# NTU-CompHydroMet-Lab/P2I-GAN-benchmark

Measured on AMD Instinct MI355X. Metric: train frames/sec (128x128x16), higher is better.
Workload: dtype f32

## Files before the change

include/p2i_hip.h:

```cpp
#ifndef P2I_HIP_H
#define P2I_HIP_H
#include <stdint.h>

#ifdef __cplusplus
extern "C" {
#endif

#define P2I_OK 0
#define P2I_EINVAL (-1)
#define P2I_ELDS (-2)

#define P2I_ACT_NONE 0
#define P2I_ACT_RELU 1
#define P2I_ACT_LEAKY 2
#define P2I_ACT_TANH 3

int p2i_abi_version(void);
const char* p2i_last_error(void);

typedef struct {
  int B, Cin, Cout;
  int Ti, Hi, Wi;
  int To, Ho, Wo;
  int kt, kh, kw;
  int st, sh, sw;
  int pt, ph, pw;
} p2i_conv_desc;

int p2i_conv_fwd(const p2i_conv_desc* d, const float* x, const float* wp, const float* bias,
                 const float* residual, float* y, int act, void* stream);
int p2i_conv_dgrad(const p2i_conv_desc* d, const float* dy, const float* y_act, int act,
                   const float* wp_d, const float* dx_add, const float* mask_y, int mask_act,
                   float* dx, void* stream);
int p2i_conv_wgrad(const p2i_conv_desc* d, const float* x, const float* dy, const float* y_act,
                   int act, float* dwp, float* dbias, void* stream);
int p2i_conv_wgrad_ws(const p2i_conv_desc* d, const float* x, const float* dy, const float* y_act, int act, float* dwp,
                      float* dbias, float* ws, int64_t ws_floats, void* stream);
int p2i_conv_fwd_x6(const p2i_conv_desc* d, const float* x, const float* wp, uint16_t* wsplit, const float* bias,
                    const float* residual, float* y, int act, void* stream);
int p2i_conv_dgrad_x6(const p2i_conv_desc* d, const float* dy, const float* wp_d, uint16_t* wsplit, const float* dx_add,
                      const float* mask_y, int mask_act, float* dx, void* stream);
int p2i_x6_split(const float* wp, uint16_t* wb, int ntaps, int K, int Mpad, void* stream);
int p2i_x6_split_batched(const float* const* wp, uint16_t* const* wb, const int* ntaps, const int* K, const int* Mpad, int n,
                         void* stream);
int p2i_x6c_would_take(const p2i_conv_desc* d, int dgrad, int act);
int p2i_conv_fwd_x6s(const p2i_conv_desc* d, const float* x, const float* wp, const uint16_t* wb_layer, int ntaps_w,
                     const float* bias, const float* residual, float* y, int act, void* stream);
int p2i_conv_dgrad_x6s(const p2i_conv_desc* d, const float* dy, const float* wp_d, const uint16_t* wb_layer, int ntaps_w,
                       const float* dx_add, const float* mask_y, int mask_act, float* dx, void* stream);
int p2i_conv_last_plan(int* out6);
int p2i_fast_div_magic(int d, uint32_t* magic);
int p2i_wgrad_last_plan(int* out4);

int p2i_doconv_fold_fwd(const float* W, const float* D, const float* D_diag, int O, int I, int groups,
                        int ksz, int identity_rep, float* wp_f, float* wp_d, void* stream);
int p2i_doconv_fold_bwd(const float* dwp_f, const float* W, const float* D, const float* D_diag,
                        int O, int I, int groups, int ksz, float* dW, float* dD, void* stream);

int p2i_doconv_fold_fwd_batched(const float* const* W, const float* const* D, const float* const* D_diag, int n, int O, int I,
                                float* const* wp_f, float* const* wp_d, void* stream);
int p2i_doconv_fold_bwd_batched(const float* const* dwp_f, const float* const* W, const float* const* D,
                                const float* const* D_diag, int n, int O, int I, float* const* dW, float* const* dD,
                                void* stream);

int p2i_weight_pack(const float* w, int O, int I, int ntaps, const float* inv_div_ptr,
                    float* wp_f, float* wp_d, void* stream);
int p2i_weight_unpack_grad(const float* dwp_f, int O, int I, int ntaps, const float* w_orig,
                           const float* sigma_ptr, const float* u, const float* v, float* scratch,
                           float* dw, void* stream);

int p2i_weight_pack_batched(const float* const* w, const int* O, const int* I, const int* ntaps, const float* const* inv_div,
                            float* const* wp_f, float* const* wp_d, int n, void* stream);
int p2i_weight_unpack_grad_batched(const float* const* dwp_f, const int* O, const int* I, const int* ntaps,
                                   const float* const* w_orig, const float* const* sigma, const float* const* u,
                                   const float* const* v, float* dots, float* const* dw, int n, void* stream);

int p2i_weight_unpack_grad_batched_acc(const float* const* dwp_f, const int* O, const int* I, const int* ntaps,
                                       const float* const* w_orig, const float* const* sigma, const float* const* u,
                                       const float* const* v, float* dots, float* const* dw, int n, int accumulate, void* stream);

int p2i_spectral_norm(const float* w, int O, int K, float* u, float* v, int training, float* sigma,
                      float* scratch, void* stream);

int p2i_spectral_norm_batched(const float* const* w, const int* O, const int* K, float* const* u, float* const* v,
                              int training, float* const* sigma, float* const* scratch, float* const* u_snap,
                              float* const* v_snap, int n, void* stream);

int p2i_attn_fwd(const float* x, const float* w0, const float* b0, const float* w1, const float* b1,
                 float* out, int B, int T, int HW, void* stream);
int p2i_attn_bwd(const float* x, const float* w0, const float* b0, const float* w1, const float* b1,
                 const float* dout, float* dw0, float* db0, float* dw1, float* db1,
                 int B, int T, int HW, void* stream);

int p2i_idw_fwd(const float* vals_src, const float* mask, const float* grid_x, const float* grid_y,
                const float* grid_z, float* out, int32_t* pt_pos, int32_t* pt_count, int32_t* frame_count,
                int32_t* row_start, float* pt_xyzn, int32_t* sel_idx, float* sel_w, int B, int T, int H, int W, float tau,
                void* stream);
int p2i_idw_fwd_ws(const float* vals_src, const float* mask, const float* grid_x, const float* grid_y,
                   const float* grid_z, float* out, int32_t* pt_pos, int32_t* pt_count, int32_t* frame_count,
                   int32_t* row_start, float* pt_xyzn, int32_t* sel_idx, float* sel_w, int32_t* amb, int B, int T, int H, int W,
                   float tau, void* stream);
int p2i_idw_bwd(const float* dout, const int32_t* pt_pos, const int32_t* pt_count, const int32_t* sel_idx,
                const float* sel_w, float* dvals_src, int B, int T, int H, int W, void* stream);

int p2i_pooldup_fwd(const float* x, float* y, int B, int C, int H, int W, void* stream);
int p2i_pooldup_bwd(const float* x, const float* dy, float* dx, int B, int C, int H, int W, void* stream);

int p2i_upmod_fwd(const float* x, const float* pos, float* u, int B, int C, int S, int S2w , void* stream);
int p2i_upmod_fwd_ba(const float* v, const float* pos, const float* bias, int act, float* u, int B, int C, int S, int S2w, void* stream);
int p2i_upmod_bwd(const float* x, const float* pos, const float* du, float* dx, float* dpos,
                  int B, int C, int S, int S2w, void* stream);

int p2i_dtail_fwd(const float* out2d, const float* out3d, const float* alpha2d, float* fused,
                  int B, int H2, int W2, int T3, int H3, int W3, void* stream);
int p2i_dtail_bwd(const float* out2d, const float* alpha2d, const float* dfused, float* dout2d,
                  float* dout3d, float* dalpha2d, int B, int H2, int W2, int T3, int H3, int W3, void* stream);

int p2i_recloss(const float* pred, const float* target, float k1_alpha, float* out3, float* dpred,
                float* scratch, int B, int T, int HW, void* stream);
int p2i_gan_loss(const float* logits_a, const float* logits_b, int n, int loss_type, int mode,
                 float weight, float real_label, float fake_label, float* loss, float* dlogits_a,
                 float* dlogits_b, void* stream);

int p2i_adam(float* p, const float* g, float* m, float* v, int64_t n, float lr, float beta1,
             float beta2, float eps, int step, void* stream);

int p2i_assemble_batch(const uint8_t* frames_u8, const uint8_t* mask_u8, int64_t mask_numel, float* frames,
                       float* masked, float* masks, int B, int T, int H, int W, void* stream);

int p2i_window_gather(const float* a, const float* b , float* wa, float* wb, int L, int64_t HW, int w0, int nw, int win,
                      int step, void* stream);
int p2i_window_mean(const float* pred_windows, float* out, int L, int64_t HW, int nwin, int win, int step, float scale, void* stream);

// ... 78 lines not shown
```

p2i-gan-benchmark_amd/csrc/conv.hip:

```cpp
#include "conv_dma.h"

namespace p2i {


template <int MB, int NPIX, int WAVES_M, int CK>
__global__ __launch_bounds__(256) void patch_gemm_kernel(const PatchGeom g) {
  extern __shared__ __attribute__((aligned(16))) float smem[];
  constexpr int WAVES_N = 4 / WAVES_M;
  constexpr int TM = MB / (32 * WAVES_M);
  constexpr int TN = NPIX / (32 * WAVES_N);
  static_assert(TM >= 1 && TN >= 1, "tile too small");
  float* lw = smem;
  float* lp = smem + g.ntaps * CK * MB;

  const int tid = threadIdx.x, lane = tid & 63, wave = tid >> 6;
  const int wm = wave / WAVES_N, wn = wave % WAVES_N;
  const int l31 = lane & 31, lhi = lane >> 5;

  int tile = blockIdx.x;
  const int tw = tile % g.ntw; tile /= g.ntw;
  const int th = tile % g.nth; tile /= g.nth;
  const int tt = tile % g.ntt;
  const int tb = tile / g.ntt;
  const int j0b = tb << g.ljb, j0t = tt << g.ljt, j0h = th << g.ljh, j0w = tw << g.ljw;
// ... 76 lines not shown
        for (int i = 0; i < TM; ++i)
#pragma unroll
          for (int f = 0; f < TN; ++f)
            acc[i][f] = __builtin_amdgcn_mfma_f32_32x32x2f32(a[i], bv[f], acc[i][f], 0, 0, 0);
      }
    }
  }

  const int dHW = g.dH * g.dW;
#pragma unroll
  for (int f = 0; f < TN; ++f) {
    const int pix = (wn * TN + f) * 32 + l31;
    const int gw = j0w + (pix & JWm);
    const int gh = j0h + ((pix >> g.ljw) & JHm);
    const int gt = j0t + ((pix >> (g.ljw + g.ljh)) & JTm);
    const int gb = j0b + (pix >> (g.ljw + g.ljh + g.ljt));
    const bool pv = gb < g.B && gt < g.nT && gh < g.nH && gw < g.nW;
    const int sp = (gt * g.oT + g.pT) * dHW + (gh * g.oH + g.pH) * g.dW + gw * g.oW + g.pW;
#pragma unroll
    for (int i = 0; i < TM; ++i) {
#pragma unroll
      for (int r = 0; r < 16; ++r) {
        const int o = o0 + (wm * TM + i) * 32 + (r & 3) + 8 * (r >> 2) + 4 * lhi;
        if (pv && o < g.Cm) {
          float v = acc[i][f][r];
          if (g.bias) v += g.bias[o];
          v = act_apply(v, g.act_epi);
          const size_t di = ((size_t)(gb * g.Cm + o)) * g.dT * dHW + sp;
          if (g.res) v += g.res[di];
          if (g.mask_y) v = act_grad(v, g.mask_y[di], g.mask_act);
          g.dst[di] = v;
        }
      }
    }
  }
}


typedef void (*patch_fn)(const PatchGeom);
template <int MB, int NPIX, int WM, int CK>
static int launch_patch(const PatchGeom& g, dim3 grid, size_t lds, hipStream_t s) {
  auto k = patch_gemm_kernel<MB, NPIX, WM, CK>;
  static bool attr_set = false;
  if (!attr_set) {
    (void)hipFuncSetAttribute((const void*)k, hipFuncAttributeMaxDynamicSharedMemorySize, 160 * 1024);
    attr_set = true;
  }
  P2I_LAUNCH(k, grid, dim3(256), lds, s, g);
  return launch_status();
}

static int dispatch_patch_dma(const TileCfg& c, int KG, const PatchGeom& g, dim3 grid, size_t lds, hipStream_t s) {
  int rc = dispatch_patch_dma_g0(c, KG, g, grid, lds, s);
  if (rc == -1) rc = dispatch_patch_dma_g1(c, KG, g, grid, lds, s);
  if (rc == -1) rc = dispatch_patch_dma_g2(c, KG, g, grid, lds, s);
  if (rc == -1) rc = dispatch_patch_dma_g3(c, KG, g, grid, lds, s);
  if (rc != -1) return rc;
  set_error("no DMA kernel instance for tile cfg %d %d %d %d kg %d", c.MB, c.NPIX, c.WM, c.CK, KG);
  return P2I_EINVAL;
}

static int dispatch_patch(const TileCfg& c, const PatchGeom& g, dim3 grid, size_t lds, hipStream_t s) {
#define P2I_CASE(mb_, npix_, wm_, ck_) \
  if (c.MB == mb_ && c.NPIX == npix_ && c.WM == wm_ && c.CK == ck_) return launch_patch<mb_, npix_, wm_, ck_>(g, grid, lds, s);
  P2I_CASE(128, 256, 2, 8)
  P2I_CASE(64, 256, 1, 8)
  P2I_CASE(64, 128, 2, 8)
  P2I_CASE(32, 128, 1, 8)
  P2I_CASE(128, 256, 2, 4)
  P2I_CASE(64, 256, 1, 4)
  P2I_CASE(64, 128, 2, 4)
  P2I_CASE(32, 128, 1, 4)
  P2I_CASE(128, 256, 2, 2)
  P2I_CASE(64, 256, 1, 2)
  P2I_CASE(64, 128, 2, 2)
  P2I_CASE(32, 128, 1, 2)
#undef P2I_CASE
  set_error("no kernel instance for tile cfg %d %d %d %d", c.MB, c.NPIX, c.WM, c.CK);
  return P2I_EINVAL;
}


static thread_local int g_last_plan[6] = {0, 0, 0, 0, 0, 0};

static int run_patch_gemm(PatchGeom g, const ClassSpec& cs, hipStream_t s);

static int run_patch_gemm_classes(PatchGeom g, const ClassSpec* css, int ncls, hipStream_t s) {
  if (g.src_y != nullptr || ncls > MAX_CLASSES) return 1;
  if (const X6Ctx& xc = x6_ctx(); xc.wb != nullptr) {
    bool all = true;
    for (int q = 0; q < ncls && all; ++q) all = run_patch_gemm_x6c(g, css[q], xc.wb, xc.ntaps_w, nullptr, s, true) == 0;
    if (all) {
      for (int q = 0; q < ncls; ++q)
        if (const int rc = run_patch_gemm_x6c(g, css[q], xc.wb, xc.ntaps_w, g_last_plan, s)) return rc == 1 ? P2I_EINVAL : rc;
      return P2I_OK;
    }
  }
  const ClassSpec& c0s = css[0];
  g.mT = c0s.mT; g.mH = c0s.mH; g.mW = c0s.mW;
  g.oT = c0s.oT; g.oH = c0s.oH; g.oW = c0s.oW;
  int lo[MAX_CLASSES][3], rng[3] = {0, 0, 0}, mx[3] = {0, 0, 0}, max_taps = 0;
  long long total_pix = 0;
  for (int q = 0; q < ncls; ++q) {
    const ClassSpec& cs = css[q];
    int hi[3] = {0, 0, 0};
    lo[q][0] = lo[q][1] = lo[q][2] = 0;
    for (int i = 0; i < cs.ntaps; ++i) {
      const int d[3] = {cs.dt[i], cs.dh[i], cs.dw[i]};
      for (int k = 0; k < 3; ++k) {
        if (i == 0 || d[k] < lo[q][k]) lo[q][k] = d[k];
        if (i == 0 || d[k] > hi[k]) hi[k] = d[k];
      }
    }
    for (int k = 0; k < 3; ++k) if (hi[k] - lo[q][k] > rng[k]) rng[k] = hi[k] - lo[q][k];
    if (cs.nT > mx[0]) mx[0] = cs.nT;
    if (cs.nH > mx[1]) mx[1] = cs.nH;
    if (cs.nW > mx[2]) mx[2] = cs.nW;
    if (cs.ntaps > max_taps) max_taps = cs.ntaps;
    total_pix += (long long)g.B * (cs.nT > 0 ? cs.nT : 0) * (cs.nH > 0 ? cs.nH : 0) * (cs.nW > 0 ? cs.nW : 0);
  }
  if (mx[0] <= 0 || mx[1] <= 0 || mx[2] <= 0) return P2I_OK;
  if (max_taps == 0) max_taps = 1;
  g.ntaps = max_taps;
  static const int cand[5][3] = {{128, 256, 2}, {64, 256, 1}, {128, 128, 2}, {64, 128, 2}, {32, 128, 1}};
  int best = -1, best_ck = 0;
  long long best_score = -1;
  PatchGeom bg = g;
  size_t best_lds = 0;
  dim3 best_grid;
  for (int ci = 0; ci < 5; ++ci) {
    const int MBc = cand[ci][0], NP = cand[ci][1];
    if (MBc > 32 && g.Cm <= MBc / 2) continue;
    int jb, jt, jh, jw;
    pick_tile_dims(NP, g.B, mx[0], mx[1], mx[2], jb, jt, jh, jw);
    PatchGeom t = g;
    t.ljb = ilog2(jb); t.ljt = ilog2(jt); t.ljh = ilog2(jh); t.ljw = ilog2(jw);
    t.eT = (jt - 1) * g.mT + rng[0] + 1;
    t.eH = patch_extent_div((jh - 1) * g.mH + rng[1] + 1);
    t.eW = (jw - 1) * g.mW + rng[2] + 1;
    bool same_lo_w = true;
    for (int q = 1; q < ncls; ++q) same_lo_w = same_lo_w && lo[q][2] == lo[0][2];
    t.v4 = (conv_v4_on() && same_lo_w && (g.sW & 3) == 0 && ((jw * g.mW) & 3) == 0) ? 1 : 0;
    t.v4sh = 0;
    if (t.v4) {
      t.v4sh = ((lo[0][2] % 4) + 4) % 4;
      t.eW = (t.eW + t.v4sh + 3) & ~3;
      t.eW4 = t.eW >> 2;
    }
    if (!t.v4) t.eW = patch_extent_div(t.eW);
    t.eWp = t.eW;
    t.eth = t.eT * t.eH;
    t.rpc = jb * t.eth;
    t.CSl = t.rpc * t.eW;
    t.CS = t.CSl;
    t.G4 = t.CSl >> 2;
    const int force_ck16 = P2I_ENV_ONCE("P2I_CONV_CK16", 0);
    for (int CKc = ((max_taps <= 4 || ((force_ck16 || g.Ck >= 256) && max_taps == 9 && MBc <= 64)) ? 16 : 8); CKc >= 2; CKc >>= 1) {
      if (g.Ck >= CKc ? (g.Ck % CKc != 0) : (CKc != 2 && g.Ck * 2 <= CKc)) continue;
      if (CKc == 2 && !(MBc == 64 && NP == 128) && !(MBc == 32)) continue;
      if ((CKc == 4 || CKc == 16) && MBc == 128 && NP == 128) continue;
      const int PT = CKc * t.CSl;
      if (PT >= 65536 || t.CSl >= 65536) continue;
      const int PTp = t.v4 ? (((PT >> 2) + 63) & ~63) * 4 : (PT + 63) & ~63;
      const int nwrows = max_taps * CKc;
      const size_t WSZ = (size_t)((nwrows * (MBc / 4) + 63) & ~63) * 4;
      const size_t lds = sizeof(float) * (((nwrows + 63) & ~63) + (size_t)PTp + 2 * (WSZ + PTp));
      if (lds > 160 * 1024) continue;
      const long long nb = (long long)ceil_div(g.Cm, MBc) * ((total_pix + NP - 1) / NP);
      long long score = (nb >= 256 ? 1000000000ll : nb * 1000000ll) + (long long)MBc * NP * 10 + CKc + (lds <= 80 * 1024 ? 5 : 0);
      if (score > best_score) {
        best_score = score; best = ci; best_ck = CKc; best_lds = lds;
        bg = t; bg.PT = PT;
        bg.ntt = ceil_div(mx[0], jt); bg.nth = ceil_div(mx[1], jh); bg.ntw = ceil_div(mx[2], jw);
        best_grid = dim3((unsigned)(ceil_div(g.B, jb) * bg.ntt * bg.nth * bg.ntw), (unsigned)ceil_div(g.Cm, MBc), (unsigned)ncls);
      }
      break;
    }
  }
  const unsigned long long sbytes = 4ull * g.B * g.Ck * g.sT * g.sH * g.sW;
  if (best < 0 || sbytes >= 0xF0000000ull) return 1;
  TileCfg c{cand[best][0], cand[best][1], cand[best][2], best_ck};
  P2I_REQUIRE(magic_u16_ok(bg.CSl) && magic_u16_ok(bg.eW) && magic_u16_ok(bg.rpc) && magic_u16_ok(bg.eth) && magic_u16_ok(bg.eH) &&
              (!bg.v4 || (magic_u16_ok(bg.G4) && (bg.eW4 == 1 || magic_u16_ok(bg.eW4)))),
              "conv planner: offset-table divisor outside [2, 65535] (%d %d %d %d %d)", bg.CSl, bg.eW, bg.rpc, bg.eth, bg.eH);
  bg.mg_csl = magic_u16(bg.CSl); bg.mg_ew = magic_u16(bg.eW);
  bg.mg_rpc = magic_u16(bg.rpc); bg.mg_eth = magic_u16(bg.eth); bg.mg_eh = magic_u16(bg.eH);
  if (bg.v4) { bg.mg_g4 = magic_u16(bg.G4); bg.mg_ew4 = magic_u16(bg.eW4); }
  bg.src_bytes = (unsigned)sbytes;
  bg.wp_bytes = g.wp_bytes;
  bg.nclass = ncls;
  for (int q = 0; q < ncls; ++q) {
    const ClassSpec& cs = css[q];
    ClassGeom& cgm = bg.cls[q];
    cgm.nT = cs.nT; cgm.nH = cs.nH; cgm.nW = cs.nW;
    cgm.pT = cs.pT; cgm.pH = cs.pH; cgm.pW = cs.pW;
    cgm.bT = lo[q][0]; cgm.bH = lo[q][1]; cgm.bW = lo[q][2];
    cgm.ntaps = cs.ntaps;
    for (int i = 0; i < cs.ntaps; ++i) {
      cgm.tap_w[i] = cs.tw[i];
      cgm.tap_off[i] = ((cs.dt[i] - lo[q][0]) * bg.eH + (cs.dh[i] - lo[q][1])) * bg.eW + (cs.dw[i] - lo[q][2]);
    }
  }
  bg.nT = css[0].nT; bg.nH = css[0].nH; bg.nW = css[0].nW;
  bg.pT = css[0].pT; bg.pH = css[0].pH; bg.pW = css[0].pW;
  bg.bT = lo[0][0]; bg.bH = lo[0][1]; bg.bW = lo[0][2];
  for (int i = 0; i < css[0].ntaps; ++i) { bg.tap_w[i] = bg.cls[0].tap_w[i]; bg.tap_off[i] = bg.cls[0].tap_off[i]; }
  if (bg.v4) {
    bg.bW -= bg.v4sh;
    for (int i = 0; i < css[0].ntaps; ++i) bg.tap_off[i] += bg.v4sh;
    for (int q = 0; q < ncls; ++q) {
      bg.cls[q].bW -= bg.v4sh;
      for (int i = 0; i < css[q].ntaps; ++i) bg.cls[q].tap_off[i] += bg.v4sh;
    }
  }
  if (ncls == 1) bg.ntaps = css[0].ntaps;
  const long long nb = (long long)best_grid.x * best_grid.y * best_grid.z;
  const int acc_regs = (c.MB / 32) * (c.NPIX / 32) / 4 * 16;
  const size_t red_bytes = (size_t)4 * acc_regs * 64 * 4;
  const int kg27 = P2I_ENV_ONCE("P2I_CONV_KG27", 1);
  const bool kg_27 = kg27 && max_taps == 27 && c.CK == 4 && ncls == 1;
  const int KG = ((nb <= 320 || (c.CK == 16 && max_taps == 9) || kg_27) && (c.CK >= 8 || kg_27) && c.MB <= 64 && red_bytes <= best_lds) ? 2 : 1;
  g_last_plan[0] = c.MB; g_last_plan[1] = c.NPIX; g_last_plan[2] = c.WM; g_last_plan[3] = c.CK;
  g_last_plan[4] = ncls > 1 ? 0 : ((max_taps == 9 && (c.CK <= 8 || KG == 2)) ? 9 : (max_taps == 1 ? 1 : ((max_taps == 27 && (c.CK == 4 || (c.CK < 4 && KG == 1))) ? 27 : 0)));
  g_last_plan[5] = KG;
  return dispatch_patch_dma(c, KG, bg, best_grid, best_lds, s);
}

static int run_patch_gemm(PatchGeom g, const ClassSpec& cs, hipStream_t s) {
  if (cs.nT <= 0 || cs.nH <= 0 || cs.nW <= 0) return P2I_OK;
  {
    const int rc = run_patch_gemm_classes(g, &cs, 1, s);
    if (rc != 1) return rc;
  }
  g.nT = cs.nT; g.nH = cs.nH; g.nW = cs.nW;
  g.mT = cs.mT; g.mH = cs.mH; g.mW = cs.mW;
  g.oT = cs.oT; g.oH = cs.oH; g.oW = cs.oW; g.pT = cs.pT; g.pH = cs.pH; g.pW = cs.pW;
  g.ntaps = cs.ntaps;
  g.nclass = 1;
  int lo[3] = {0, 0, 0}, hi[3] = {0, 0, 0};
  for (int i = 0; i < cs.ntaps; ++i) {
    const int d[3] = {cs.dt[i], cs.dh[i], cs.dw[i]};
    for (int k = 0; k < 3; ++k) {
      if (i == 0 || d[k] < lo[k]) lo[k] = d[k];
      if (i == 0 || d[k] > hi[k]) hi[k] = d[k];
    }
  }
  g.bT = lo[0]; g.bH = lo[1]; g.bW = lo[2];

  TileCfg c;
  c.CK = (g.Ck == 1) ? 2 : (cs.ntaps > 9 ? 4 : 8);
  if (g.Ck < c.CK && g.Ck > 1) c.CK = (g.Ck >= 4) ? 4 : 2;
  c.MB = g.Cm > 64 ? 128 : (g.Cm > 32 ? 64 : 32);
  c.NPIX = 256;
  const long long total_pix = (long long)g.B * cs.nT * cs.nH * cs.nW;
  auto nblocks = [&](const TileCfg& t) { return (long long)ceil_div(g.Cm, t.MB) * ((total_pix + t.NPIX - 1) / t.NPIX); };
  const long long want = 512;
  while (nblocks(c) < want) {
    if (c.MB == 128) { c.MB = 64; continue; }
    if (c.NPIX == 256) { c.NPIX = 128; continue; }
    if (c.MB == 64 && g.Cm > 32) { c.MB = 32; continue; }
    break;
  }
  if (c.MB == 128) { c.NPIX = 256; c.WM = 2; }
  else if (c.MB == 64) { c.WM = (c.NPIX == 256) ? 1 : 2; }
  else { c.NPIX = 128; c.WM = 1; }

  for (int attempt = 0; attempt < 4; ++attempt) {
    int jb, jt, jh, jw;
    pick_tile_dims(c.NPIX, g.B, cs.nT, cs.nH, cs.nW, jb, jt, jh, jw);
    g.ljb = ilog2(jb); g.ljt = ilog2(jt); g.ljh = ilog2(jh); g.ljw = ilog2(jw);
    g.eT = (jt - 1) * cs.mT + (hi[0] - lo[0]) + 1;
    g.eH = patch_extent_div((jh - 1) * cs.mH + (hi[1] - lo[1]) + 1);
    g.eW = (jw - 1) * cs.mW + (hi[2] - lo[2]) + 1;
    g.eWp = g.eW | 1;
    g.eth = g.eT * g.eH;
    g.rpc = jb * g.eth;
    g.CS = g.rpc * g.eWp;
    P2I_REQUIRE(magic_u16_ok(g.eH) && magic_u16_ok(g.eth) && g.rpc >= 2, "conv planner: staging divisor below 2 (%d %d %d)", g.rpc, g.eth, g.eH);
    g.mg_rpc = magic_u16(g.rpc); g.mg_eth = magic_u16(g.eth); g.mg_eh = magic_u16(g.eH);
    const size_t lds = sizeof(float) * ((size_t)cs.ntaps * c.CK * c.MB + (size_t)c.CK * g.CS);
    if (lds > 160 * 1024 || c.CK * g.rpc >= 65536) {
      if (c.CK > 2) { c.CK /= 2; continue; }
      if (c.NPIX == 256) { c.NPIX = 128; c.WM = (c.MB == 64) ? 2 : (c.MB == 128 ? 2 : 1); if (c.MB == 128) c.MB = 64; continue; }
      set_error("conv tile does not fit LDS (%zu bytes)", lds);
      return P2I_ELDS;
    }
    for (int i = 0; i < cs.ntaps; ++i) {
      g.tap_w[i] = cs.tw[i];
      g.tap_off[i] = ((cs.dt[i] - lo[0]) * g.eH + (cs.dh[i] - lo[1])) * g.eWp + (cs.dw[i] - lo[2]);
    }
    g.ntt = ceil_div(cs.nT, jt); g.nth = ceil_div(cs.nH, jh); g.ntw = ceil_div(cs.nW, jw);
    const int ntb = ceil_div(g.B, jb);
    dim3 grid((unsigned)(ntb * g.ntt * g.nth * g.ntw), (unsigned)ceil_div(g.Cm, c.MB));
    g_last_plan[0] = c.MB; g_last_plan[1] = c.NPIX; g_last_plan[2] = c.WM; g_last_plan[3] = c.CK; g_last_plan[4] = -1; g_last_plan[5] = 0;
    return dispatch_patch(c, g, grid, lds, s);
  }
  set_error("conv tile selection failed");
  return P2I_ELDS;
}

}

using namespace p2i;

#ifdef P2I_STAMP
namespace p2i { __device__ unsigned long long* p2i_stamp_buf = nullptr; }
extern "C" int p2i_debug_set_stamp(unsigned long long* buf) {
  return (int)hipMemcpyToSymbol(HIP_SYMBOL(p2i::p2i_stamp_buf), &buf, sizeof(buf));
}
#endif

extern "C" int p2i_conv_last_plan(int* out6) {
  if (!out6) return P2I_EINVAL;
  for (int i = 0; i < 6; ++i) out6[i] = g_last_plan[i];
  return P2I_OK;
}

extern "C" int p2i_fast_div_magic(int d, uint32_t* magic) {
  P2I_REQUIRE(magic != nullptr, "null pointer");
  P2I_REQUIRE(magic_u16_ok(d), "fast_div: no 32-bit multiplier for divisor %d (2 <= d < 65536)", d);
  *magic = magic_u16(d);
  return P2I_OK;
}

extern "C" int p2i_conv_fwd(const p2i_conv_desc* d, const float* x, const float* wp, const float* bias,
                            const float* residual, float* y, int act, void* stream) {
  if (int e = check_desc(d)) return e;
  P2I_REQUIRE(x && wp && y, "null pointer");
  if (d->Cin == 1 && residual == nullptr && x6_ctx().wb == nullptr) {
    const int rc = c1_fwd(d, x, wp, bias, y, act, (hipStream_t)stream);
    if (rc != 1) { g_last_plan[0] = 32; g_last_plan[1] = 64; g_last_plan[2] = 1; g_last_plan[3] = 2; g_last_plan[4] = 27; g_last_plan[5] = 1; return rc; }
  }
  if (d->Cout == 1 && residual == nullptr) {
    const int rc = o1_fwd(d, x, wp, bias, y, act, (hipStream_t)stream);
    if (rc != 1) { g_last_plan[0] = 1; g_last_plan[1] = 64; g_last_plan[2] = 8; g_last_plan[3] = 1; g_last_plan[4] = 9; g_last_plan[5] = 3; return rc; }
  }
  PatchGeom g{};
  g.src = x; g.src_y = nullptr; g.wp = wp; g.bias = bias; g.res = residual; g.dst = y; g.act_epi = act; g.act_pro = P2I_ACT_NONE;
  g.B = d->B; g.Ck = d->Cin; g.Cm = d->Cout; g.CmPad = (d->Cout + 31) / 32 * 32;
  g.wp_bytes = 4u * (unsigned)(d->kt * d->kh * d->kw) * g.Ck * g.CmPad;
  g.sT = d->Ti; g.sH = d->Hi; g.sW = d->Wi; g.dT = d->To; g.dH = d->Ho; g.dW = d->Wo;
  ClassSpec cs{};
  cs.nT = d->To; cs.nH = d->Ho; cs.nW = d->Wo;
  cs.mT = d->st; cs.mH = d->sh; cs.mW = d->sw;
  cs.oT = cs.oH = cs.oW = 1; cs.pT = cs.pH = cs.pW = 0;
  int n = 0;
  for (int a = 0; a < d->kt; ++a)
    for (int b = 0; b < d->kh; ++b)
      for (int c = 0; c < d->kw; ++c) {
        cs.tw[n] = (short)n; cs.dt[n] = a - d->pt; cs.dh[n] = b - d->ph; cs.dw[n] = c - d->pw; ++n;
      }
  cs.ntaps = n;
  return run_patch_gemm(g, cs, (hipStream_t)stream);
}

extern "C" int p2i_conv_dgrad(const p2i_conv_desc* d, const float* dy, const float* y_act, int act,
                              const float* wp_d, const float* dx_add, const float* mask_y, int mask_act,
                              float* dx, void* stream) {
  if (int e = check_desc(d)) return e;
  P2I_REQUIRE(dy && wp_d && dx, "null pointer");
  PatchGeom g{};
  g.src = dy; g.src_y = y_act; g.wp = wp_d; g.bias = nullptr; g.res = dx_add; g.dst = dx; g.act_epi = P2I_ACT_NONE; g.act_pro = y_act ? act : P2I_ACT_NONE;
  g.mask_y = mask_y; g.mask_act = mask_y ? mask_act : P2I_ACT_NONE;
  P2I_REQUIRE(!(mask_y && y_act), "dgrad: use either the act'(y) prologue or the epilogue mask");
  if (d->Cin == 1 && !y_act && d->kt * d->kh * d->kw * d->Cout * 4 <= 64 * 1024) {
    g_last_plan[0] = 1; g_last_plan[1] = 256; g_last_plan[2] = 1; g_last_plan[3] = 1; g_last_plan[4] = d->kt * d->kh * d->kw; g_last_plan[5] = 4;
    return c1_dgrad(d, dy, wp_d, dx_add, mask_y, mask_act, dx, (hipStream_t)stream);
  }
  g.B = d->B; g.Ck = d->Cout; g.Cm = d->Cin; g.CmPad = (d->Cin + 31) / 32 * 32;
  g.wp_bytes = 4u * (unsigned)(d->kt * d->kh * d->kw) * g.Ck * g.CmPad;
  g.sT = d->To; g.sH = d->Ho; g.sW = d->Wo; g.dT = d->Ti; g.dH = d->Hi; g.dW = d->Wi;
  ClassSpec css[MAX_CLASSES];
  int ncls = 0;
  const bool mergeable = d->st * d->sh * d->sw <= MAX_CLASSES;
  for (int ct = 0; ct < d->st; ++ct)
    for (int chh = 0; chh < d->sh; ++chh)
      for (int cw = 0; cw < d->sw; ++cw) {
        ClassSpec cs{};
        cs.nT = (d->Ti - ct + d->st - 1) / d->st;
        cs.nH = (d->Hi - chh + d->sh - 1) / d->sh;
        cs.nW = (d->Wi - cw + d->sw - 1) / d->sw;
        cs.mT = cs.mH = cs.mW = 1;
        cs.oT = d->st; cs.oH = d->sh; cs.oW = d->sw; cs.pT = ct; cs.pH = chh; cs.pW = cw;
        int n = 0;
        for (int a = 0; a < d->kt; ++a) {
          if ((ct + d->pt - a) % d->st) continue;
          for (int b = 0; b < d->kh; ++b) {
            if ((chh + d->ph - b) % d->sh) continue;
            for (int c = 0; c < d->kw; ++c) {
              if ((cw + d->pw - c) % d->sw) continue;
              cs.tw[n] = (short)((a * d->kh + b) * d->kw + c);
              cs.dt[n] = (ct + d->pt - a) / d->st; cs.dh[n] = (chh + d->ph - b) / d->sh; cs.dw[n] = (cw + d->pw - c) / d->sw;
              ++n;
            }
          }
        }
        cs.ntaps = n;
// ... 83 lines not shown
```

p2i-gan-benchmark_amd/csrc/conv_common.h:

```cpp
#pragma once
#include "common.h"

namespace p2i {

typedef float f32x16 __attribute__((ext_vector_type(16)));
constexpr int MAX_TAPS = 27;

typedef __attribute__((address_space(3))) void lds_void;
typedef int v4i32 __attribute__((ext_vector_type(4)));

__device__ __forceinline__ v4i32 make_rsrc(const void* p, unsigned bytes) {
  const unsigned long long a = (unsigned long long)p;
  v4i32 r;
  r[0] = __builtin_amdgcn_readfirstlane((int)(unsigned)a);
  r[1] = __builtin_amdgcn_readfirstlane((int)(unsigned)(a >> 32));
  r[2] = __builtin_amdgcn_readfirstlane((int)bytes);
  r[3] = 0x00020000;
  return r;
}
__device__ __forceinline__ unsigned lds_base(const float* shared_array) {
  return (unsigned)(size_t)(const lds_void*)shared_array;
}
__device__ __forceinline__ void dma_b32(const v4i32 rsrc, unsigned lds_addr, int voff, int soff) {
  const unsigned la = __builtin_amdgcn_readfirstlane(lds_addr);
// ... 139 lines not shown
      v[0] = acc0[r]; v[1] = acc1[r];
      if (res) { v[0] += rv[k][0]; v[1] += rv[k][1]; }
      if (mask_y) { v[0] = act_grad(v[0], mv[k][0], mask_act); v[1] = act_grad(v[1], mv[k][1], mask_act); }
      if (ok[k]) {
        if (atomic_out) { atomicAdd(dst + di[k], v[0]); atomicAdd(dst + di[k] + 1, v[1]); }
        else *reinterpret_cast<f32x2e*>(dst + di[k]) = v;
      }
    }
    __builtin_amdgcn_sched_barrier(0);
  }
}

inline bool conv_v4_on() { return P2I_ENV_ONCE("P2I_CONV_V4", 1) != 0; }

static inline void pick_tile_dims(int NPIX, int B, int nT, int nH, int nW, int& jb, int& jt, int& jh, int& jw) {
  jw = pow2_ceil(nW); if (jw > 32) jw = 32;
  int rem = NPIX / jw;
  jh = pow2_ceil(nH); if (jh > rem) jh = rem;
  rem /= jh;
  jt = pow2_ceil(nT); if (jt > rem) jt = rem;
  rem /= jt;
  jb = rem;
  (void)B;
}


static inline int check_desc(const p2i_conv_desc* d) {
  P2I_REQUIRE(d != nullptr, "null conv desc");
  P2I_REQUIRE(d->B > 0 && d->Cin > 0 && d->Cout > 0, "bad channel/batch dims");
  P2I_REQUIRE(d->kt >= 1 && d->kh >= 1 && d->kw >= 1 && d->kt * d->kh * d->kw <= MAX_TAPS, "kernel taps > %d", MAX_TAPS);
  P2I_REQUIRE(d->st >= 1 && d->sh >= 1 && d->sw >= 1, "bad stride");
  P2I_REQUIRE(d->To == (d->Ti + 2 * d->pt - d->kt) / d->st + 1, "To inconsistent");
  P2I_REQUIRE(d->Ho == (d->Hi + 2 * d->ph - d->kh) / d->sh + 1, "Ho inconsistent");
  P2I_REQUIRE(d->Wo == (d->Wi + 2 * d->pw - d->kw) / d->sw + 1, "Wo inconsistent");
  const long long nin = (long long)d->B * d->Cin * d->Ti * d->Hi * d->Wi;
  const long long nout = (long long)d->B * d->Cout * d->To * d->Ho * d->Wo;
  P2I_REQUIRE(nin < (1ll << 31) && nout < (1ll << 31), "tensor too large for 32-bit indexing");
  return P2I_OK;
}


struct ClassGeom {
  int nT, nH, nW, pT, pH, pW, bT, bH, bW, ntaps;
  short tap_w[MAX_TAPS];
  int tap_off[MAX_TAPS];
};
constexpr int MAX_CLASSES = 8;

struct PatchGeom {
  const float* src;
  const float* src_y;
  const float* wp;
  const float* bias;
  const float* res;
  float* dst;
  int act_epi;
  int act_pro;
  int B, Ck, Cm, CmPad;
  int sT, sH, sW;
  int dT, dH, dW;
  int nT, nH, nW;
  int mT, mH, mW;
  int oT, oH, oW;
  int pT, pH, pW;
  int bT, bH, bW;
  int eT, eH, eW, eWp;
  int ljb, ljt, ljh, ljw;
  int ntt, nth, ntw;
  int ntaps;
  int CS;
  int rpc, eth;
  unsigned mg_rpc, mg_eth, mg_eh;
  short tap_w[MAX_TAPS];
  int tap_off[MAX_TAPS];
  const float* mask_y;
  int mask_act;
  int CSl;
  int PT;
  unsigned src_bytes, wp_bytes;
  unsigned mg_csl, mg_ew;
  int v4, v4sh;
  int eW4, G4;
  unsigned mg_g4, mg_ew4;
  const uint16_t* wb;
  unsigned wb_bytes;
  int ntaps_w;
  int TG, NTP, R;
  int ksplit;
  int pair_w;
  int nclass;
  ClassGeom cls[MAX_CLASSES];
};

struct ClassSpec {
  int nT, nH, nW;
  int mT, mH, mW;
  int oT, oH, oW, pT, pH, pW;
  int ntaps;
  short tw[MAX_TAPS];
  int dt[MAX_TAPS], dh[MAX_TAPS], dw[MAX_TAPS];
};

struct X6Ctx { const uint16_t* wb; int ntaps_w; };
X6Ctx& x6_ctx();

int run_patch_gemm_x6c(const PatchGeom& g, const ClassSpec& cs, const uint16_t* wb, int ntaps_w, int* plan6, hipStream_t s, bool dry = false);
int run_patch_gemm_x6c_fused(const PatchGeom& g, const ClassSpec* css, int ncls, const uint16_t* wb, int ntaps_w, int* plan6, hipStream_t s, bool dry = false);
bool x6c_would_take(const p2i_conv_desc* d, bool dgrad, int act_epi);

int run_patch_gemm_fused(PatchGeom g, const ClassSpec* css, int ncls, int* plan6, hipStream_t s);

int c1_dgrad(const p2i_conv_desc* d, const float* dy, const float* wp_d, const float* add, const float* mask_y, int mask_act,
             float* dx, hipStream_t s);
int c1_wgrad(const p2i_conv_desc* d, const float* x, const float* dy, float* dwp, float* dbias, hipStream_t s);
int c1_fwd(const p2i_conv_desc* d, const float* x, const float* wp, const float* bias, float* y, int act, hipStream_t s);
int o1_fwd(const p2i_conv_desc* d, const float* x, const float* wp, const float* bias, float* y, int act, hipStream_t s);

}
```

p2i-gan-benchmark_amd/csrc/conv_dma.h:

```cpp
#pragma once
#include "conv_common.h"

namespace p2i {

struct TileCfg { int MB, NPIX, WM, CK; };

#ifdef P2I_STAMP
extern __device__ unsigned long long* p2i_stamp_buf;
#endif

template <int MB, int NPIX, int WAVES_M, int CK, int NT, int KG>
__global__ __launch_bounds__(256 * KG) void patch_gemm_dma_kernel(const PatchGeom g) {
  extern __shared__ __attribute__((aligned(16))) float smem[];
  constexpr int WAVES_N = 4 / WAVES_M;
  constexpr int TM = MB / (32 * WAVES_M);
  constexpr int TN = NPIX / (32 * WAVES_N);
  constexpr int V = MB / 4;
  const bool multi = g.nclass > 1;
  const ClassGeom& cg = g.cls[multi ? blockIdx.z : 0];
  const int c_nT = multi ? cg.nT : g.nT, c_nH = multi ? cg.nH : g.nH, c_nW = multi ? cg.nW : g.nW;
  const int c_pT = multi ? cg.pT : g.pT, c_pH = multi ? cg.pH : g.pH, c_pW = multi ? cg.pW : g.pW;
  const int c_bT = multi ? cg.bT : g.bT, c_bH = multi ? cg.bH : g.bH, c_bW = multi ? cg.bW : g.bW;
  const int c_ntaps = multi ? cg.ntaps : g.ntaps;
  const short* c_tap_w = multi ? cg.tap_w : g.tap_w;
  const int* c_tap_off = multi ? cg.tap_off : g.tap_off;
  const int nwrows = g.ntaps * CK;
  const int WSZ = ((nwrows * V + 63) & ~63) * 4;
  const int PT4p = ((g.PT >> 2) + 63) & ~63;
  const int PTp = g.v4 ? PT4p * 4 : (g.PT + 63) & ~63;
  int* wtab = reinterpret_cast<int*>(smem);
  const int wtab_sz = (nwrows + 63) & ~63;
  int* ptab = wtab + wtab_sz;
  float* buf0 = smem + wtab_sz + PTp;
  const int BUFSZ = WSZ + PTp;

  constexpr int NTH = 256 * KG;
#ifdef P2I_STAMP
  unsigned long long st_entry;
  asm volatile("s_memtime %0\n\ts_waitcnt lgkmcnt(0)" : "=s"(st_entry) :: "memory");
#endif
  const int tid = threadIdx.x, lane = tid & 63, wave = (tid >> 6) & 3, kg = tid >> 8;
  const int wm = wave / WAVES_N, wn = wave % WAVES_N;
  const int l31 = lane & 31, lhi = lane >> 5;

  int tile = blockIdx.x;
  const int tw = tile % g.ntw; tile /= g.ntw;
  const int th = tile % g.nth; tile /= g.nth;
  const int tt = tile % g.ntt;
  const int tb = tile / g.ntt;
  const int j0b = tb << g.ljb, j0t = tt << g.ljt, j0h = th << g.ljh, j0w = tw << g.ljw;
  const int o0 = blockIdx.y * MB;
  const int JWm = (1 << g.ljw) - 1, JHm = (1 << g.ljh) - 1, JTm = (1 << g.ljt) - 1;
  const int sHW = g.sH * g.sW;
  const int src_t0 = j0t * g.mT + c_bT, src_h0 = j0h * g.mH + c_bH, src_w0 = j0w * g.mW + c_bW;

  for (int r = tid; r < wtab_sz; r += NTH) {
    int off = -4;
    if (r < nwrows) {
      const int tap = r / CK, c = r - tap * CK;
      if (tap < c_ntaps && c < g.Ck && o0 < g.CmPad) off = ((c_tap_w[tap] * g.Ck + c) * g.CmPad + o0) * 4;
    }
    wtab[r] = off;
  }
  if (g.v4) {
    for (int e = tid; e < PT4p; e += NTH) {
      int off = -16;
      if (e < (g.PT >> 2)) {
        const int c = fast_div(e, g.mg_g4);
        int rem = e - c * g.G4;
        const int row = g.eW4 == 1 ? rem : fast_div(rem, g.mg_ew4);
        const int g4 = rem - row * g.eW4;
        const int jb = fast_div(row, g.mg_eth);
        int r2 = row - jb * g.eth;
        const int et = fast_div(r2, g.mg_eh);
        const int eh = r2 - et * g.eH;
        const int b = j0b + jb, t = src_t0 + et, h = src_h0 + eh, w = src_w0 + 4 * g4;
        if (b < g.B && c < g.Ck && (unsigned)t < (unsigned)g.sT && (unsigned)h < (unsigned)g.sH && (unsigned)w < (unsigned)g.sW)
          off = ((((b * g.Ck + c) * g.sT + t) * sHW) + h * g.sW + w) * 4;
      }
      ptab[e] = off;
    }
  } else
  for (int e = tid; e < PTp; e += NTH) {
    int off = -4;
    if (e < g.PT) {
      const int c = fast_div(e, g.mg_csl);
      int rem = e - c * g.CSl;
      const int row = fast_div(rem, g.mg_ew);
      const int ew = rem - row * g.eW;
      const int jb = fast_div(row, g.mg_eth);
      int r2 = row - jb * g.eth;
      const int et = fast_div(r2, g.mg_eh);
      const int eh = r2 - et * g.eH;
      const int b = j0b + jb, t = src_t0 + et, h = src_h0 + eh, w = src_w0 + ew;
      if (b < g.B && c < g.Ck && (unsigned)t < (unsigned)g.sT && (unsigned)h < (unsigned)g.sH && (unsigned)w < (unsigned)g.sW)
        off = ((((b * g.Ck + c) * g.sT + t) * sHW) + h * g.sW + w) * 4;
    }
    ptab[e] = off;
  }

  int lane_base[TN];
#pragma unroll
  for (int f = 0; f < TN; ++f) {
    const int pix = (wn * TN + f) * 32 + l31;
    const int jw = pix & JWm;
    const int jh = (pix >> g.ljw) & JHm;
    const int jt = (pix >> (g.ljw + g.ljh)) & JTm;
    const int jb = pix >> (g.ljw + g.ljh + g.ljt);
    lane_base[f] = ((jb * g.eT + jt * g.mT) * g.eH + jh * g.mH) * g.eW + jw * g.mW + lhi * g.CSl;
  }
  f32x16 acc[TM][TN];
#pragma unroll
  for (int i = 0; i < TM; ++i)
#pragma unroll
    for (int f = 0; f < TN; ++f)
#pragma unroll
      for (int r = 0; r < 16; ++r) acc[i][f][r] = 0.f;

  const v4i32 rs_src = make_rsrc(g.src, g.src_bytes);
  const v4i32 rs_w = make_rsrc(g.wp, g.wp_bytes);
  const unsigned smem_la = lds_base(smem);
  const int buf0_off = (int)(buf0 - smem);
  const int chan_bytes = g.sT * sHW * 4;
  const int wbase = tid & ~63;
  const int nwv = nwrows * V;
  __syncthreads();

  constexpr int RW = 10, RP = 4;
  const int nwq = (((nwv + 63) & ~63) + NTH - 1) / NTH;
  const int npq = g.v4 ? (PT4p + NTH - 1) / NTH : RP + 1;
  const bool reg_issue = nwq <= RW && npq <= RP;
  int wv[RW], pv[RP];
  if (reg_issue) {
#pragma unroll
    for (int i = 0; i < RW; ++i) {
      const int f = i * NTH + tid;
      int voff = -4;
      if (i < nwq && f < nwv) {
        const int row = f / V, col4 = f - row * V;
        const int base = wtab[row];
        voff = base < 0 ? -4 : base + col4 * 16;
      }
      wv[i] = voff;
    }
#pragma unroll
    for (int i = 0; i < RP; ++i) {
      const int e = i * NTH + tid;
      pv[i] = (i < npq && e < PT4p) ? ptab[e] : -16;
    }
  }
  auto issue = [&](int c0, int bufoff) {
    const int w_soff = c0 * g.CmPad * 4;
    if (reg_issue) {
      const int p_soff = c0 * chan_bytes, pbo = bufoff + WSZ;
#pragma unroll
      for (int i = 0; i < RW; ++i)
        if (i < nwq && i * NTH + wbase < ((nwv + 63) & ~63))
          dma_b128(rs_w, smem_la + 4u * (bufoff + (i * NTH + wbase) * 4), wv[i], w_soff);
#pragma unroll
      for (int i = 0; i < RP; ++i)
        if (i < npq && i * NTH + wbase < PT4p)
          dma_b128(rs_src, smem_la + 4u * (pbo + (i * NTH + wbase) * 4), pv[i], p_soff);
      return;
    }
    for (int f0 = 0; f0 < nwv; f0 += NTH) {
      const int f = f0 + tid;
      int voff = -4;
      if (f < nwv) {
        const int row = f / V, col4 = f - row * V;
        const int base = wtab[row];
        voff = base < 0 ? -4 : base + col4 * 16;
      }
      if (f0 + wbase < ((nwv + 63) & ~63))
        dma_b128(rs_w, smem_la + 4u * (bufoff + (f0 + wbase) * 4), voff, w_soff);
    }
    const int pbo = bufoff + WSZ;
    const int p_soff = c0 * chan_bytes;
    if (g.v4) {
      for (int e0 = 0; e0 < PT4p; e0 += NTH) {
        const int e = e0 + tid;
        const int voff = e < PT4p ? ptab[e] : -16;
        if (e0 + wbase < PT4p)
          dma_b128(rs_src, smem_la + 4u * (pbo + (e0 + wbase) * 4), voff, p_soff);
      }
    } else
    for (int e0 = 0; e0 < PTp; e0 += NTH) {
      const int e = e0 + tid;
      const int voff = e < PTp ? ptab[e] : -4;
      if (e0 + wbase < PTp)
        dma_b32(rs_src, smem_la + 4u * (pbo + e0 + wbase), voff, p_soff);
    }
  };
// ... 177 lines not shown
```

p2i-gan-benchmark_amd/p2igan_bench/_hip.py:

```python
from __future__ import annotations

import ctypes as C
import os

_LIB_PATH = os.path.join(os.path.dirname(os.path.abspath(__file__)), "_lib", "libp2i_hip.so")
_lib = None

ACT_NONE, ACT_RELU, ACT_LEAKY, ACT_TANH = 0, 1, 2, 3


class ConvDesc(C.Structure):
    _fields_ = [(n, C.c_int) for n in
                ("B", "Cin", "Cout", "Ti", "Hi", "Wi", "To", "Ho", "Wo", "kt", "kh", "kw",
                 "st", "sh", "sw", "pt", "ph", "pw")]


_P = C.c_void_p
_I = C.c_int
_F = C.c_float
_L = C.c_int64
_D = C.POINTER(ConvDesc)

SIGNATURES = {
    "p2i_conv_fwd": [_D, _P, _P, _P, _P, _P, _I, _P],
    "p2i_conv_dgrad": [_D, _P, _P, _I, _P, _P, _P, _I, _P, _P],
    "p2i_conv_wgrad": [_D, _P, _P, _P, _I, _P, _P, _P],
    "p2i_conv_wgrad_ws": [_D, _P, _P, _P, _I, _P, _P, _P, _L, _P],
    "p2i_conv_fwd_x6": [_D, _P, _P, _P, _P, _P, _P, _I, _P],
    "p2i_conv_dgrad_x6": [_D, _P, _P, _P, _P, _P, _I, _P, _P],
    "p2i_x6_split": [_P, _P, _I, _I, _I, _P],
    "p2i_x6_split_batched": [_P, _P, _P, _P, _P, _I, _P],
    "p2i_x6c_would_take": [_D, _I, _I],
    "p2i_conv_fwd_x6s": [_D, _P, _P, _P, _I, _P, _P, _P, _I, _P],
    "p2i_conv_dgrad_x6s": [_D, _P, _P, _P, _I, _P, _P, _I, _P, _P],
    "p2i_conv_last_plan": [C.POINTER(C.c_int)],
    "p2i_wgrad_last_plan": [C.POINTER(C.c_int)],
    "p2i_fast_div_magic": [_I, C.POINTER(C.c_uint32)],
    "p2i_doconv_fold_fwd": [_P, _P, _P, _I, _I, _I, _I, _I, _P, _P, _P],
    "p2i_doconv_fold_bwd": [_P, _P, _P, _P, _I, _I, _I, _I, _P, _P, _P],
    "p2i_doconv_fold_fwd_batched": [_P, _P, _P, _I, _I, _I, _P, _P, _P],
    "p2i_doconv_fold_bwd_batched": [_P, _P, _P, _P, _I, _I, _I, _P, _P, _P],
    "p2i_weight_pack": [_P, _I, _I, _I, _P, _P, _P, _P],
    "p2i_weight_pack_batched": [_P, _P, _P, _P, _P, _P, _P, _I, _P],
    "p2i_weight_unpack_grad_batched": [_P, _P, _P, _P, _P, _P, _P, _P, _P, _P, _I, _P],
    "p2i_weight_unpack_grad_batched_acc": [_P, _P, _P, _P, _P, _P, _P, _P, _P, _P, _I, _I, _P],
    "p2i_weight_unpack_grad": [_P, _I, _I, _I, _P, _P, _P, _P, _P, _P, _P],
    "p2i_spectral_norm": [_P, _I, _I, _P, _P, _I, _P, _P, _P],
    "p2i_spectral_norm_batched": [_P, _P, _P, _P, _P, _I, _P, _P, _P, _P, _I, _P],
    "p2i_attn_fwd": [_P, _P, _P, _P, _P, _P, _I, _I, _I, _P],
    "p2i_attn_bwd": [_P, _P, _P, _P, _P, _P, _P, _P, _P, _P, _I, _I, _I, _P],
    "p2i_idw_fwd": [_P, _P, _P, _P, _P, _P, _P, _P, _P, _P, _P, _P, _P, _I, _I, _I, _I, _F, _P],
    "p2i_idw_fwd_ws": [_P, _P, _P, _P, _P, _P, _P, _P, _P, _P, _P, _P, _P, _P, _I, _I, _I, _I, _F, _P],
    "p2i_idw_bwd": [_P, _P, _P, _P, _P, _P, _I, _I, _I, _I, _P],
    "p2i_pooldup_fwd": [_P, _P, _I, _I, _I, _I, _P],
    "p2i_pooldup_bwd": [_P, _P, _P, _I, _I, _I, _I, _P],
    "p2i_upmod_fwd": [_P, _P, _P, _I, _I, _I, _I, _P],
    "p2i_window_gather": [_P, _P, _P, _P, _I, _L, _I, _I, _I, _I, _P],
    "p2i_window_mean": [_P, _P, _I, _L, _I, _I, _I, _F, _P],
    "p2i_upmod_fwd_ba": [_P, _P, _P, _I, _P, _I, _I, _I, _I, _P],
    "p2i_upmod_bwd": [_P, _P, _P, _P, _P, _I, _I, _I, _I, _P],
    "p2i_dtail_fwd": [_P, _P, _P, _P, _I, _I, _I, _I, _I, _I, _P],
    "p2i_dtail_bwd": [_P, _P, _P, _P, _P, _P, _I, _I, _I, _I, _I, _I, _P],
    "p2i_recloss": [_P, _P, _F, _P, _P, _P, _I, _I, _I, _P],
    "p2i_gan_loss": [_P, _P, _I, _I, _I, _F, _F, _F, _P, _P, _P, _P],
    "p2i_adam": [_P, _P, _P, _P, _L, _F, _F, _F, _F, _I, _P],
    "p2i_adam_dev": [_P, _P, _P, _P, _L, _F, _F, _F, _F, _P, _P, _P],
    "p2i_metrics_pointwise": [_P, _P, _L, C.POINTER(C.c_float), _I, _I, _P, _P, _P, _P],
    "p2i_metrics_fss": [_P, _I, _I, _I, _I, C.POINTER(C.c_int), _I, _P, _P, _P],
    "p2i_assemble_batch": [_P, _P, _L, _P, _P, _P, _I, _I, _I, _I, _P],
    "p2i_axpy": [_P, _P, _F, _L, _P],
    "p2i_add2": [_P, _P, _P, _L, _P],
    "p2i_zero": [_P, _L, _P],
    "p2i_act_bwd": [_P, _P, _I, _P, _L, _P],
    "p2i_bias_grad": [_P, _P, _I, _P, _I, _I, _L, _P],
    "p2i_act_bwd_bias": [_P, _P, _I, _P, _P, _I, _I, _L, _P],
    "p2i_det_workspace": [_P, _L, _P, _I],
    "p2i_x6_split_planes": [_P, _P, _I, _I, _L, _P],
    "p2i_x6_next_source_planes": [_P],
    "p2i_event_record": [_I, _P],
    "p2i_event_wait": [_I, _P],
    "p2i_tape_begin": [_P],
    "p2i_tape_end": [C.POINTER(C.c_void_p)],
    "p2i_tape_info": [_P, C.POINTER(C.c_int)],
    "p2i_tape_replay": [_P, _P],
    "p2i_tape_free": [_P],
    "p2i_stdk_basis": [_P, _P, _I, _I, _I, _P, _P],
    "p2i_stdk_select": [_P, _P, _I, _I, _I, _P, _P, _P],
    "p2i_stdk_layer1_fwd": [_P, _P, _P, _P, _P, _I, _I, _I, _I, _I, _I, _P, _P, _P, _P, _P],
    "p2i_stdk_mlp_fwd": [_P, _P, _P, _P, _P, _P, _P, _P, _I, _I, _P, _P],
    "p2i_stdk_bwd_workspace": [_I, _I, C.POINTER(C.c_int64)],
    "p2i_stdk_mlp_bwd": [_P] * 8 + [_I, _I] + [_P] * 13,
    "p2i_stdk_layer1_bwd": [_P, _P, _P, _P, _P, _I, _I, _I, _I, _I, _I, _P, _P, _P, _I, _P, _P, _P],
    "p2i_exp1_transform": [_P, _I, _L, _I, _P, _P],
    "p2i_exp1_workspace": [_I, _I, _I, C.POINTER(C.c_int64)],
    "p2i_exp1_accumulate": [_P, _I, _I, _I, _I, _I, _P, _I, _I, _I, _I, _I, _I, _I, _I, _P, _I, _P,
                            C.POINTER(C.c_double), _I, _I, _P, _P, _P, _P, _P, _P],
    "p2i_exp1_merge": [_P, _L, _P, _P],
    "p2i_exp1_hist": [_P, _P, _I, _I, _P, _P, _P, _P, _P],
    "p2i_exp1_ssim": [_P, _P, _I, _I, _P, _P, _P, _P],
    "p2i_exp1_finalize": [_P, C.POINTER(C.c_double), _I, _I, _P, _P, _P, _P, _P, _P, _P, _P],
    "p2i_exp3_accumulate": [_P, _I, _I, _I, _I, _I, _P, _I, _I, _I, _I, _I, _I, _I, _P, _P, _I, _P, _P, _P, _P],
    "p2i_exp3_truth_hist": [_P, _I, _I, _I, _I, _I, _I, _I, _P, _I, _P, _P],
    "p2i_exp3_scan": [_P, _L, _P, _P],
    "p2i_exp3_gather": [_P, _I, _I, _I, _I, _I, _P, _I, _I, _I, _I, _I, _I, _I, _P, _I, _P, _L, _P, _I, _P, _P, _P],
    "p2i_exp3_nse": [_P, _P, _I, _P, _I, _P, _P],
}


def lib_path() -> str:
    return _LIB_PATH


def load():
    global _lib
    if _lib is not None:
        return _lib
    if not os.path.exists(_LIB_PATH):
        raise RuntimeError(
# ... 18 lines not shown
```

Measured before the change: 11700.

## Deinterleave stride-2 patch staging in LDS to avoid bank conflicts

For single-class stride-2 (mW==2) convolutions, the planner checks whether the lanes of a wavefront reading the staged input patch from LDS collide on the same banks. If they do, it stores the patch with even and odd columns split into two halves, picks a row pitch that gives conflict-free reads, and remaps tap offsets and the DMA gather to match. This is meant to remove LDS bank conflicts in the patch-GEMM inner loop. In exchange it turns off the v4 vectorised gather path and adds a per-element column remap during the fill.

```diff
diff --git a/include/p2i_hip.h b/include/p2i_hip.h
--- a/include/p2i_hip.h
+++ b/include/p2i_hip.h
@@ -49,6 +49,7 @@
 int p2i_conv_dgrad_x6s(const p2i_conv_desc* d, const float* dy, const float* wp_d, const uint16_t* wb_layer, int ntaps_w,
                        const float* dx_add, const float* mask_y, int mask_act, float* dx, void* stream);
 int p2i_conv_last_plan(int* out6);
+int p2i_conv_last_image(int* out3);
 int p2i_fast_div_magic(int d, uint32_t* magic);
 int p2i_wgrad_last_plan(int* out4);
 
diff --git a/p2i-gan-benchmark_amd/csrc/conv.hip b/p2i-gan-benchmark_amd/csrc/conv.hip
--- a/p2i-gan-benchmark_amd/csrc/conv.hip
+++ b/p2i-gan-benchmark_amd/csrc/conv.hip
@@ -182,6 +182,18 @@
 
 
 static thread_local int g_last_plan[6] = {0, 0, 0, 0, 0, 0};
+static thread_local int g_last_image[3] = {0, 0, 0};
+
+static int b_read_ways(const PatchGeom& t, int eW, int lW) {
+  int cnt[32] = {0}, worst = 0;
+  for (int l = 0; l < 32; ++l) {
+    const int jw = l & ((1 << t.ljw) - 1), jh = (l >> t.ljw) & ((1 << t.ljh) - 1), jt = (l >> (t.ljw + t.ljh)) & ((1 << t.ljt) - 1);
+    const int jb = l >> (t.ljw + t.ljh + t.ljt);
+    const int a = ((jb * t.eT + jt * t.mT) * t.eH + jh * t.mH) * eW + jw * lW;
+    if (++cnt[a & 31] > worst) worst = cnt[a & 31];
+  }
+  return worst;
+}
 
 static int run_patch_gemm(PatchGeom g, const ClassSpec& cs, hipStream_t s);
 
@@ -280,6 +292,18 @@
   const unsigned long long sbytes = 4ull * g.B * g.Ck * g.sT * g.sH * g.sW;
   if (best < 0 || sbytes >= 0xF0000000ull) return 1;
   TileCfg c{cand[best][0], cand[best][1], cand[best][2], best_ck};
+  bg.img = 0; bg.eWh = 0;
+  if (ncls == 1 && g.mW == 2 && b_read_ways(bg, bg.eW, 2) > 1) {
+    const int half = ((1 << bg.ljw) - 1) + (rng[2] + 2) / 2, nodd = ((1 << bg.ljw) - 1) + (rng[2] + 1) / 2;
+    for (int pitch = half + nodd < 2 ? 2 : half + nodd; pitch <= bg.eW; ++pitch)
+      if (b_read_ways(bg, pitch, 1) == 1) {
+        bg.img = 1; bg.eWh = half; bg.v4 = 0; bg.v4sh = 0;
+        bg.eW = bg.eWp = pitch;
+        bg.CSl = bg.CS = bg.rpc * pitch;
+        bg.PT = best_ck * bg.CSl;
+        break;
+      }
+  }
   P2I_REQUIRE(magic_u16_ok(bg.CSl) && magic_u16_ok(bg.eW) && magic_u16_ok(bg.rpc) && magic_u16_ok(bg.eth) && magic_u16_ok(bg.eH) &&
               (!bg.v4 || (magic_u16_ok(bg.G4) && (bg.eW4 == 1 || magic_u16_ok(bg.eW4)))),
               "conv planner: offset-table divisor outside [2, 65535] (%d %d %d %d %d)", bg.CSl, bg.eW, bg.rpc, bg.eth, bg.eH);
@@ -298,7 +322,8 @@
     cgm.ntaps = cs.ntaps;
     for (int i = 0; i < cs.ntaps; ++i) {
       cgm.tap_w[i] = cs.tw[i];
-      cgm.tap_off[i] = ((cs.dt[i] - lo[q][0]) * bg.eH + (cs.dh[i] - lo[q][1])) * bg.eW + (cs.dw[i] - lo[q][2]);
+      const int dwr = cs.dw[i] - lo[q][2];
+      cgm.tap_off[i] = ((cs.dt[i] - lo[q][0]) * bg.eH + (cs.dh[i] - lo[q][1])) * bg.eW + (bg.img ? (dwr & 1) * bg.eWh + (dwr >> 1) : dwr);
     }
   }
   bg.nT = css[0].nT; bg.nH = css[0].nH; bg.nW = css[0].nW;
@@ -322,6 +347,7 @@
   const int KG = ((nb <= 320 || (c.CK == 16 && max_taps == 9) || kg_27) && (c.CK >= 8 || kg_27) && c.MB <= 64 && red_bytes <= best_lds) ? 2 : 1;
   g_last_plan[0] = c.MB; g_last_plan[1] = c.NPIX; g_last_plan[2] = c.WM; g_last_plan[3] = c.CK;
   g_last_plan[4] = ncls > 1 ? 0 : ((max_taps == 9 && (c.CK <= 8 || KG == 2)) ? 9 : (max_taps == 1 ? 1 : ((max_taps == 27 && (c.CK == 4 || (c.CK < 4 && KG == 1))) ? 27 : 0)));
+  g_last_image[0] = bg.img; g_last_image[1] = bg.eW; g_last_image[2] = bg.v4;
   g_last_plan[5] = KG;
   return dispatch_patch_dma(c, KG, bg, best_grid, best_lds, s);
 }
@@ -413,6 +439,12 @@
 extern "C" int p2i_conv_last_plan(int* out6) {
   if (!out6) return P2I_EINVAL;
   for (int i = 0; i < 6; ++i) out6[i] = g_last_plan[i];
+  return P2I_OK;
+}
+
+extern "C" int p2i_conv_last_image(int* out3) {
+  if (!out3) return P2I_EINVAL;
+  for (int i = 0; i < 3; ++i) out3[i] = g_last_image[i];
   return P2I_OK;
 }
 
diff --git a/p2i-gan-benchmark_amd/csrc/conv_common.h b/p2i-gan-benchmark_amd/csrc/conv_common.h
--- a/p2i-gan-benchmark_amd/csrc/conv_common.h
+++ b/p2i-gan-benchmark_amd/csrc/conv_common.h
@@ -245,6 +245,7 @@
   int v4, v4sh;
   int eW4, G4;
   unsigned mg_g4, mg_ew4;
+  int img, eWh;
   const uint16_t* wb;
   unsigned wb_bytes;
   int ntaps_w;
diff --git a/p2i-gan-benchmark_amd/csrc/conv_dma.h b/p2i-gan-benchmark_amd/csrc/conv_dma.h
--- a/p2i-gan-benchmark_amd/csrc/conv_dma.h
+++ b/p2i-gan-benchmark_amd/csrc/conv_dma.h
@@ -92,13 +92,15 @@
       int r2 = row - jb * g.eth;
       const int et = fast_div(r2, g.mg_eh);
       const int eh = r2 - et * g.eH;
-      const int b = j0b + jb, t = src_t0 + et, h = src_h0 + eh, w = src_w0 + ew;
+      const int wc = !g.img ? ew : (ew < g.eWh ? 2 * ew : (ew < 2 * g.eWh ? 2 * (ew - g.eWh) + 1 : (1 << 24)));
+      const int b = j0b + jb, t = src_t0 + et, h = src_h0 + eh, w = src_w0 + wc;
       if (b < g.B && c < g.Ck && (unsigned)t < (unsigned)g.sT && (unsigned)h < (unsigned)g.sH && (unsigned)w < (unsigned)g.sW)
         off = ((((b * g.Ck + c) * g.sT + t) * sHW) + h * g.sW + w) * 4;
     }
     ptab[e] = off;
   }
 
+  const int lW = g.img ? 1 : g.mW;
   int lane_base[TN];
 #pragma unroll
   for (int f = 0; f < TN; ++f) {
@@ -107,7 +109,7 @@
     const int jh = (pix >> g.ljw) & JHm;
     const int jt = (pix >> (g.ljw + g.ljh)) & JTm;
     const int jb = pix >> (g.ljw + g.ljh + g.ljt);
-    lane_base[f] = ((jb * g.eT + jt * g.mT) * g.eH + jh * g.mH) * g.eW + jw * g.mW + lhi * g.CSl;
+    lane_base[f] = ((jb * g.eT + jt * g.mT) * g.eH + jh * g.mH) * g.eW + jw * lW + lhi * g.CSl;
   }
   f32x16 acc[TM][TN];
 #pragma unroll
diff --git a/p2i-gan-benchmark_amd/p2igan_bench/_hip.py b/p2i-gan-benchmark_amd/p2igan_bench/_hip.py
--- a/p2i-gan-benchmark_amd/p2igan_bench/_hip.py
+++ b/p2i-gan-benchmark_amd/p2igan_bench/_hip.py
@@ -34,6 +34,7 @@
     "p2i_conv_fwd_x6s": [_D, _P, _P, _P, _I, _P, _P, _P, _I, _P],
     "p2i_conv_dgrad_x6s": [_D, _P, _P, _P, _I, _P, _P, _I, _P, _P],
     "p2i_conv_last_plan": [C.POINTER(C.c_int)],
+    "p2i_conv_last_image": [C.POINTER(C.c_int)],
     "p2i_wgrad_last_plan": [C.POINTER(C.c_int)],
     "p2i_fast_div_magic": [_I, C.POINTER(C.c_uint32)],
     "p2i_doconv_fold_fwd": [_P, _P, _P, _I, _I, _I, _I, _I, _P, _P, _P],
```

New measurement: 11440. -2.2%, worse.
